# marmotlab/DCMRTA

Hardware: AMD Instinct MI355X
Metric: env_steps_per_sec (higher is better)
Workload: dtype f64

## Files before the change

### dcmrta_amd/_lib.py

```python
import ctypes as C
import os

_HERE = os.path.dirname(os.path.abspath(__file__))
LIB_PATH = os.environ.get("DCMRTA_HIP_LIB") or os.path.join(_HERE, "libdcmrta_hip.so")
HEADER_PATH = os.path.join(os.path.dirname(_HERE), "include", "dcmrta_env.h")

ABI_VERSION = 5
FOLLOWER_COLS = 4
MAX_MEMBERS = 5
MAX_MEMBERS_WIDE = 16
PARAM_NO_GROUPING, PARAM_AUTO_RESET, PARAM_STRICT_MASK, PARAM_WIDE_MEMBERS = 1, 2, 4, 8
PARAM_RENEW_SIZES = 16
POLICY_RANDOM, POLICY_FIRST, POLICY_NEAREST = 0, 1, 2
MAX_AGENTS = 128
MAX_TASKS = 1023

FLAG_DONE, FLAG_FINISHED, FLAG_TRUNCATED, FLAG_BAD_ACTION, FLAG_OVERFLOW, FLAG_BAD_LEADER, FLAG_TYPE_ERROR = 1, 2, 4, 8, 16, 32, 64
FLAG_BAD_INSTANCE = 256
FLAG_WAIT_ORDER = 128


class DcmParams(C.Structure):
    _fields_ = [("n_envs", C.c_int32), ("n_agents", C.c_int32), ("n_tasks", C.c_int32), ("device", C.c_int32),
                ("max_waiting_time", C.c_double), ("max_time", C.c_double), ("flags", C.c_uint32),
                ("auto_reset_episodes", C.c_uint32)]


class DcmError(RuntimeError):
    pass


_vp, _i32, _i64 = C.c_void_p, C.c_int32, C.c_int64
SIGNATURES = {
    "dcm_last_error": (C.c_char_p, []),
    "dcm_abi_version": (C.c_int, []),
    "dcm_build_id": (C.c_char_p, []),
    "dcm_create": (C.c_int, [C.POINTER(DcmParams), C.POINTER(_vp)]),
    "dcm_destroy": (C.c_int, [_vp]),
    "dcm_load_instances": (C.c_int, [_vp] * 6),
    "dcm_load_instances_ragged": (C.c_int, [_vp] * 8),
    "dcm_generate_instances": (C.c_int, [_vp, _vp, _i32, _i32, _i32, _i32, _i32, C.c_double, _vp]),
    "dcm_get_instances": (C.c_int, [_vp] * 8),
    "dcm_set_instance_renewal": (C.c_int, [_vp, C.c_uint64]),
    "dcm_instance_index": (C.c_int, [_vp] * 3),
    "dcm_generator_draws": (C.c_int, [_vp, _i64, _i32, C.c_uint32, _i32, _vp, _vp, _vp]),
    "dcm_reset": (C.c_int, [_vp] * 3),
    "dcm_observe": (C.c_int, [_vp] * 8),
    "dcm_step": (C.c_int, [_vp] * 11),
    "dcm_rollout_random": (C.c_int, [_vp, _i32, _i64, _vp, _vp, _vp, _vp, _vp, _vp]),
    "dcm_rollout_policy": (C.c_int, [_vp, _i32, _i32, _i64, _vp, _vp, _vp, _vp, _vp, _vp]),
    "dcm_rollout_explore": (C.c_int, [_vp, _i32, C.c_uint64, _i32, _i64, _vp, _vp, _vp, _vp, _vp, _vp]),
# ... 57 lines not shown
```

### dcmrta_amd/batched_env.py

```python
import ctypes as C
from dataclasses import dataclass

import numpy as np
import torch

from . import _lib
from ._lib import DcmError, DcmParams, check
from .choice import explore_q32 as _choice_explore_q32

SUMMARY_COLUMNS = ("reward", "n_finished", "success_rate", "makespan", "time_cost", "waiting_time", "travel_dist",
                   "efficiency")


@dataclass
class Observation:
    agents: torch.Tensor
    tasks: torch.Tensor
    mask: torch.Tensor
    leader: torch.Tensor
    active: torch.Tensor


def _ptr(t):
    return None if t is None else C.c_void_p(t.data_ptr())
# ... 74 lines not shown
            nt = np.ascontiguousarray(n_tasks, dtype=np.int32)
            na = np.ascontiguousarray(n_agents, dtype=np.int32)
            if nt.shape != (B,) or na.shape != (B,):
                raise DcmError(f"n_agents / n_tasks must be int[{B}]")
            req_np[np.arange(T)[None, :] >= nt[:, None]] = 1
        if req_np.min() < 1 or req_np.max() > self.member_cap:
            raise DcmError(f"req must be int[{B},{T}] with values in 1..{self.member_cap} (member_cap of this env)")
        d = self._dev(depot, torch.float64)
        xy = self._dev(task_xy, torch.float64)
        rq = self._dev(req, torch.int32)
        du = self._dev(dur, torch.float64)
        if d.shape != (B, 2) or xy.shape != (B, T, 2) or du.shape != (B, T):
            raise DcmError("instance arrays have the wrong shape")
        if (n_tasks is None) != (self.n_tasks is None):
            self.graph_epoch += 1
        with torch.cuda.device(self.device):
            if n_tasks is None:
                check(self._lib.dcm_load_instances(self._h, _ptr(d), _ptr(xy), _ptr(rq), _ptr(du), self._stream()))
                self.n_agents = self.n_tasks = None
            else:
                check(self._lib.dcm_load_instances_ragged(self._h, _ptr(d), _ptr(xy), _ptr(rq), _ptr(du),
                                                          na.ctypes.data_as(C.c_void_p), nt.ctypes.data_as(C.c_void_p),
                                                          self._stream()))
                self.n_agents, self.n_tasks = na.copy(), nt.copy()
        self._instances = (d, xy, rq, du)
        return self

    @staticmethod
    def _range(r, dim):
        return (dim, dim) if r is None else (int(r[0]), int(r[1])) if isinstance(r, (tuple, list)) else (int(r), int(r))

    def generate_instances(self, seeds, agents_range=None, tasks_range=None, max_coalition_size=5, max_duration=5.0):
        B = self.B
        if isinstance(seeds, (int, np.integer)):
            seeds = np.uint64(int(seeds)) + np.arange(B, dtype=np.uint64)
        if isinstance(seeds, torch.Tensor):
            if seeds.dtype not in (torch.int64, torch.uint64):
                raise DcmError("seeds must be a uint64 / int64 tensor")
            s = seeds.to(self.device).contiguous()
        else:
            s = torch.from_numpy(np.ascontiguousarray(seeds, dtype=np.uint64).view(np.int64)).to(self.device)
        if s.numel() != B:
            raise DcmError("seeds must have one entry per env")
        (a_lo, a_hi), (t_lo, t_hi) = self._range(agents_range, self.A), self._range(tasks_range, self.T)
        ragged = not (a_lo == self.A and t_lo == self.T)
        with torch.cuda.device(self.device):
            check(self._lib.dcm_generate_instances(self._h, _ptr(s), a_lo, a_hi, t_lo, t_hi, int(max_coalition_size),
                                                   float(max_duration), self._stream()))
            if ragged != (self.n_tasks is not None):
                self.graph_epoch += 1
            if ragged:
                sizes = torch.empty((2, B), dtype=torch.int32, device=self.device)
                check(self._lib.dcm_get_instances(self._h, None, None, None, None, _ptr(sizes[0]), _ptr(sizes[1]), self._stream()))
                sizes = sizes.cpu().numpy()
                self.n_agents, self.n_tasks = sizes[0].copy(), sizes[1].copy()
            else:
                self.n_agents = self.n_tasks = None
        self._instances = (s,)
        return self

    def set_instance_renewal(self, stride):
        check(self._lib.dcm_set_instance_renewal(self._h, int(stride) % (1 << 64)))
        self.graph_epoch += 1
        return self

    def instance_index(self):
        out = torch.empty((self.B,), dtype=torch.int32, device=self.device)
        with torch.cuda.device(self.device):
            check(self._lib.dcm_instance_index(self._h, _ptr(out), self._stream()))
        return out.to(torch.int64) & 0xFFFFFFFF

    def instances(self):
        B, T, dev = self.B, self.T, self.device
# ... 346 lines not shown

    def clone_state(self):
        n = C.c_size_t()
        check(self._lib.dcm_state_bytes(self._h, C.byref(n)))
        buf = torch.empty((n.value,), dtype=torch.uint8, device=self.device)
        with torch.cuda.device(self.device):
            check(self._lib.dcm_clone_state(self._h, _ptr(buf), self._stream()))
        return buf

    def restore_state(self, buf):
        n = C.c_size_t()
        check(self._lib.dcm_state_bytes(self._h, C.byref(n)))
        if buf.numel() * buf.element_size() != n.value:
            raise DcmError(f"restore_state: the snapshot holds {buf.numel() * buf.element_size()} bytes, this env's state is {n.value} "
                           "(taken from another env, or before the batch changed between uniform and ragged)")
        with torch.cuda.device(self.device):
            check(self._lib.dcm_restore_state(self._h, _ptr(buf), self._stream()))

    def fork_from(self, src, index, seeds=None, check=False):
        if not isinstance(src, BatchedTaskEnv):
            raise DcmError("fork_from: src must be a BatchedTaskEnv")
        if (src.A, src.T, src.member_cap) != (self.A, self.T, self.member_cap):
            raise DcmError(f"fork_from: src is a {src.A}A/{src.T}T env with member_cap {src.member_cap}, this one {self.A}A/{self.T}T "
                           f"with {self.member_cap}: the record layouts must be identical")
        n = index.numel() if isinstance(index, torch.Tensor) else np.asarray(index).size
        if n != self.B:
            raise DcmError(f"fork_from: index must be int32[{self.B}], one entry per env of this handle")
        if seeds is not None:
            if isinstance(seeds, torch.Tensor):
                if seeds.dtype not in (torch.int64, torch.uint64):
                    raise DcmError("fork_from: seeds must be a uint64 / int64 tensor")
                ns = seeds.numel()
            else:
                seeds = np.ascontiguousarray(seeds, dtype=np.uint64)
                ns = seeds.size
            if ns != self.B:
                raise DcmError(f"fork_from: seeds must be uint64[{self.B}], one entry per env of this handle")
        if src.device != self.device:
            raise DcmError("fork_from: the two handles are on different devices")
        if src._h is None or self._h is None:
            raise DcmError("fork_from: a handle is closed")
        idx = self._dev(index, torch.int32).reshape(-1)
        s = None
        if seeds is not None:
            s = seeds.to(self.device).contiguous() if isinstance(seeds, torch.Tensor) else torch.from_numpy(seeds.view(np.int64)).to(self.device)
        ok = torch.empty((self.B,), dtype=torch.uint8, device=self.device) if check else None
        with torch.cuda.device(self.device):
            _lib.check(self._lib.dcm_fork_envs(self._h, src._h, _ptr(idx), _ptr(s), _ptr(ok), self._stream()))
        self._fork_args = (idx, s)
        if check:
            bad = torch.nonzero(ok == 0).flatten().cpu().numpy()
            if len(bad):
                raise DcmError(f"fork_from: {len(bad)} env(s) were refused and left untouched (first: env {int(bad[0])}, index "
                               f"{int(idx[int(bad[0])])}): the index is outside [-1, {src.B}) or, in place, its source is not its own source")
        return self

    def record_bytes(self):
        n = C.c_size_t()
        check(self._lib.dcm_record_bytes(self._h, C.byref(n)))
        return n.value


group_plan = BatchedTaskEnv.group_plan
# ... 27 lines not shown
```

### dcmrta_amd/csrc/common.hpp

```cpp
#pragma once
#include <hip/hip_runtime.h>

#include <cmath>
#include <cstdint>
#include <cstdio>
#include <cstring>
#include <new>
#include <vector>

#include "../../include/dcmrta_env.h"
#include "plan.hpp"
#include "removal_table.hpp"

namespace dcm {

constexpr int WAVE = 64;
constexpr int M = DCM_MAX_MEMBERS;
constexpr int AW_MAX = (DCM_MAX_AGENTS + 63) / 64;

struct Hdr {
    double now;
    uint64_t seed;
    uint64_t d;
    double depot_x, depot_y;
// ... 294 lines not shown
__device__ double psum(const double* a, int n) {
    if constexpr (DEPTH == 0) {
        return psum_block(a, n);
    } else {
        if (n <= 128) return psum_block(a, n);
        int n2 = n / 2;
        n2 -= n2 % 8;
        return psum<DEPTH - 1>(a, n2) + psum<DEPTH - 1>(a + n2, n - n2);
    }
}

__device__ __forceinline__ double dist2(double ax, double ay, double bx, double by) {
    const double dx = ax - bx, dy = ay - by;
    return sqrt(__builtin_fma(dy, dy, dx * dx));
}
#ifndef DCM_IEEE_DIV
__device__ __forceinline__ double over_velocity(double d) {
    const double q = d * 5.0;
    const double r = __builtin_fma(-q, 0.2, d);
    return __builtin_fma(r, 5.0, q);
}
#else
__device__ __forceinline__ double over_velocity(double d) { return d / 0.2; }
#endif

__device__ __forceinline__ void copy16(unsigned char* dst, const unsigned char* src, uint32_t bytes, int lane) {
    const uint4* s = (const uint4*)src;
    uint4* d = (uint4*)dst;
    for (uint32_t i = lane; i < bytes / 16; i += WAVE) d[i] = s[i];
}
// ... 67 lines not shown
#define LAUNCH_OK() HIP_TRY(hipGetLastError())
#define GRID(env) dim3((env)->p.n_envs), dim3(dcm::WAVE)

}

struct dcm_env {
    dcm_params p;
    int A = 0, T = 0;
    dcm::Lay L;
    dcm::KP kp;
    unsigned char* state = nullptr;
    unsigned char* gscratch = nullptr;
    double* summary = nullptr;
    uint16_t* ablog = nullptr;
    bool loaded = false, reset_done = false;
    uint64_t* inst_seeds = nullptr;
    dcm::GenArgs gen{};
    bool generated = false;
    uint64_t renew_stride = 0;
    int32_t* sizes = nullptr;
    std::vector<int32_t> sizes_host;
    int32_t* routes = nullptr;
    int32_t* route_len = nullptr;
    int32_t route_cap = 0, member_cap = 0;
    double* rmarr = nullptr;
    int32_t replay_placement = 0;
    int32_t vis[4] = {20, 20, 10, 100};
    dcm::RouteLog log{nullptr, nullptr, nullptr, 0};
    dcm::RouteLog rollout_log{nullptr, nullptr, nullptr, 0};
    dcm::BestLog best_log{nullptr, nullptr, nullptr, nullptr, nullptr};
// ... 23 lines not shown
```

### dcmrta_amd/csrc/dcmrta_env.hip

```cpp
#include <array>
#include <cstdlib>
#include <mutex>
#include <tuple>
#include <type_traits>

#include "common.hpp"
#include "np_stream.hpp"

using namespace dcm;

#if defined(DCM_TU_G) || defined(DCM_TU_P) || defined(DCM_TU_L) || defined(DCM_TU_E) || defined(DCM_TU_B) || defined(DCM_TU_A)
#define DCM_DEVICE_ONLY_TU 1
#elif !defined(DCM_SPLIT_G)
#define DCM_ONE_UNIT 1
#endif
#if defined(DCM_TU_G) || defined(DCM_ONE_UNIT)
#define DCM_HAVE_FAST_G 1
#endif
#if defined(DCM_TU_P) || defined(DCM_ONE_UNIT)
#define DCM_HAVE_POLICY 1
#endif
#if defined(DCM_TU_L) || defined(DCM_ONE_UNIT)
#define DCM_HAVE_LOG 1
#endif
// ... 1246 lines not shown
        ty[t] = task_xy[((size_t)e * T + t) * 2 + 1];
        td[t] = dur[(size_t)e * T + t];
        const int32_t r = req[(size_t)e * T + t];
        bad = bad || r < 1 || r > PC;
        ti[t] = (uint32_t)(r < 1 ? 1 : r > PC ? PC : r);
    }
    bad = __any(bad);
    if (lane == 0) {
        Hdr* h = (Hdr*)rec;
        h->depot_x = depot[2 * (size_t)e]; h->depot_y = depot[2 * (size_t)e + 1];
        h->flags = DCM_FLAG_DONE | (bad ? DCM_FLAG_BAD_INSTANCE : 0u); h->episodes = 0; h->d = 0; h->seed = 0;
        h->groups = 0; h->reserved = 0; h->max_arrival = 0.0;
    }
}

template <int CA, int CT, bool RS>
constexpr uint32_t env_kernel_lds_bytes(Lay L) { return Sim<CA, CT, RS>::lds_image_bytes(L); }

template <int CA, int CT, bool RS, int MC = M>
__global__ __launch_bounds__(WAVE) void k_reset(int A, int T, int PA, int PT, KP P, unsigned char* state, const uint64_t* seeds,
                                               double* summary, uint16_t* ablog, uint32_t mode, const int32_t* sizes,
                                               unsigned char* gscr) {
    const int e = env_of_workgroup(), lane = threadIdx.x;
    int eA, eT;
    env_dims<CA, CT, RS>(sizes, e, A, T, eA, eT);
    Sim<CA, CT, RS, false, MC> S{eA, eT, PA, PT, smem, nullptr};
    const Lay L = S.L();
    S.scr = gscr + (size_t)e * L.scratch_bytes();
    unsigned char* rec = state + (size_t)e * L.rec_bytes();
    typename Sim<CA, CT, RS, false, MC>::XY xy;
// ... 254 lines not shown
    FOR_EACH_INSTANCE(SIM_CASE)
#undef SIM_CASE
    }
    return -1;
}
template <class F>
void for_each_sim(F&& f) {
#define SIM_EACH(KIND, ...) f(SimTag<__VA_ARGS__>{});
    FOR_EACH_INSTANCE(SIM_EACH)
#undef SIM_EACH
}
template <class F>
auto with_bool(bool b, F&& f) { return b ? f(std::true_type{}) : f(std::false_type{}); }
#define DIMS(env) (env)->A, (env)->T, (env)->L.A, (env)->L.T

plan::Shape shape_of(const dcm_env* env) { return {env->A, env->T, env->sizes != nullptr, env->L.C > M, env->kp.mwt > 0.0}; }
plan::SimKind sim_of(const dcm_env* env) { return plan::sim_kind(shape_of(env)); }

struct DeviceGuard {
    int prev = -1;
    explicit DeviceGuard(int dev) { if (hipGetDevice(&prev) != hipSuccess) prev = -1; if (prev != dev) (void)hipSetDevice(dev); else prev = -1; }
    ~DeviceGuard() { if (prev >= 0) (void)hipSetDevice(prev); }
};

template <class K, class... Args, class... Tail>
void launch(K kernel, unsigned grid, unsigned lds_bytes, hipStream_t stream, const std::tuple<Args...>& args, const Tail&... tail) {
    std::apply([&](const Args&... a) { hipLaunchKernelGGL(kernel, dim3(grid), dim3(WAVE), lds_bytes, stream, a..., tail...); }, args);
}
template <class... K>
void allow_lds(int bytes, K... kernels) { ((void)hipFuncSetAttribute((const void*)kernels, hipFuncAttributeMaxDynamicSharedMemorySize, bytes), ...); }

// ... 155 lines not shown

Renew renew_args(const dcm_env* env) { return Renew{env->inst_seeds, env->renew_stride, env->gen}; }
bool renew_sizes_opted_in(const dcm_env* env) { return (env->p.flags & DCM_PARAM_RENEW_SIZES) != 0; }
plan::RenewForm launch_form(const dcm_env* env) {
    return plan::renew_form(shape_of(env), env->renew_stride != 0, renew_sizes_opted_in(env));
}
plan::RenewForm renewing_launch(dcm_env* env, void* stream) {
    const plan::RenewForm form = launch_form(env);
    if (form == plan::RenewForm::Plain) return form;
    env->init_valid = false;
    if (stream_capturing(stream)) env->captured = true;
    return form;
}
void renewal_off(dcm_env* env, bool generated) { env->generated = generated; env->renew_stride = 0; }

int launch_load(dcm_env* env, const double* depot, const double* task_xy, const int32_t* req, const double* dur, void* stream) {
    hipLaunchKernelGGL(k_load_instances, GRID(env), 0, (hipStream_t)stream, DIMS(env), env->L.C, env->state, depot, task_xy,
                       req, dur, (const int32_t*)env->sizes);
    LAUNCH_OK();
    env->loaded = true;
    env->reset_done = false;
    renewal_off(env, false);
    return DCM_OK;
}

int launch_env_status(dcm_env* env, uint32_t* flags_out, int64_t* decisions_out, double* now_out, int32_t* episodes_out, void* stream) {
    const int B = env->p.n_envs;
    hipLaunchKernelGGL(k_env_status, dim3((B + WAVE - 1) / WAVE), dim3(WAVE), 0, (hipStream_t)stream, env->L.A, env->L.T, env->L.C,
                       env->state, B, flags_out, decisions_out, now_out, episodes_out);
    LAUNCH_OK();
    return DCM_OK;
}

struct Section { void* ptr; size_t bytes; };
std::array<Section, 4> state_sections(const dcm_env* env) {
    const size_t B = (size_t)env->p.n_envs;
    const bool with_sizes = env->sizes && renew_sizes_opted_in(env);
    return {{{env->state, B * env->L.rec_bytes()}, {env->summary, B * 8 * sizeof(double)},
// ... 86 lines not shown
        return fail(DCM_ERR_STATE, "%s: the best log is set and there is no best-keeping lookahead form: clear it with "
                                   "dcm_set_best_log(env, NULL, NULL, NULL, NULL, NULL)", fn);
    return rollout_form(env, fn, FORM_LOOKAHEAD, base_policy, 0, episodes, max_decisions, max_decisions_in, agents_out, tasks_out, mask_out,
                        steps_out, stream, width, inner_out);
}
}

extern "C" {

const char* dcm_last_error(void) { return dcm::g_err; }
int dcm_abi_version(void) { return DCM_ABI_VERSION; }
#ifndef DCM_BUILD_ID
#define DCM_BUILD_ID "unknown"
#endif
const char* dcm_build_id(void) { return DCM_BUILD_ID; }
#ifdef DCM_COUNT_PATHS
int dcm_debug_path_counts(unsigned long long* out32) {
    HIP_TRY(hipDeviceSynchronize());
    HIP_TRY(hipMemcpyFromSymbol(out32, HIP_SYMBOL(g_path_counts), 32 * sizeof(unsigned long long)));
    static const unsigned long long zero[32] = {};
    HIP_TRY(hipMemcpyToSymbol(HIP_SYMBOL(g_path_counts), zero, sizeof(zero)));
    return 0;
}
#endif

int dcm_create(const dcm_params* params, dcm_env** out) {
    if (!params || !out) return fail(DCM_ERR_INVALID, "dcm_create: null argument");
    *out = nullptr;
    if (params->n_envs < 1 || params->n_agents < 1 || params->n_agents > DCM_MAX_AGENTS || params->n_tasks < 1 ||
        params->n_tasks > DCM_MAX_TASKS)
// ... 60 lines not shown
    using mc = rollout_fast_mc_family;
    allow_lds(lds, mc::plain<50, 200, true>(), mc::plain<50, 200, false>(), mc::renewing<50, 200, true>(), mc::renewing<50, 200, false>());
    dcm::allow_lds_policy(lds);
    dcm::allow_lds_log(lds);
    dcm::allow_lds_explore(lds);
    dcm::allow_lds_best(lds);
    dcm::allow_lds_lookahead(lds);
    allow_lds(lds, k_get_tasks<M>, k_get_agents<M>, k_get_tasks<MW>, k_get_agents<MW>);
    return DCM_OK;
}

int dcm_destroy(dcm_env* env) {
    if (!env) return DCM_OK;
    DeviceGuard guard(env->p.device);
    void* const owned[] = {env->state, env->summary, env->ablog, env->gscratch, env->routes, env->route_len,
                           env->rmarr, env->sizes, env->side, env->pendq, env->init, env->inst_seeds, env->la_snap};
    for (void* p : owned)
        if (p) (void)hipFree(p);
    delete env;
    return DCM_OK;
}

int dcm_load_instances(dcm_env* env, const double* depot, const double* task_xy, const int32_t* req, const double* dur,
                       void* stream) {
    CHECK_ENV(env);
    if (!depot || !task_xy || !req || !dur) return fail(DCM_ERR_INVALID, "dcm_load_instances: null array");
    DCM_TRY(dcm::drop_pending(env, stream));
    if (env->sizes) { HIP_TRY(hipFree(env->sizes)); env->sizes = nullptr; }
    return launch_load(env, depot, task_xy, req, dur, stream);
}

// ... 29 lines not shown
    DCM_TRY(dcm::drop_pending(env, stream));
    renewal_off(env, false);
    const bool uniform = agents_lo == env->A && tasks_lo == env->T;
    if (uniform && env->sizes) { HIP_TRY(hipFree(env->sizes)); env->sizes = nullptr; }
    if (!uniform && !env->sizes) HIP_TRY(hipMalloc((void**)&env->sizes, (size_t)2 * env->p.n_envs * sizeof(int32_t)));
    const size_t seed_bytes = (size_t)env->p.n_envs * sizeof(uint64_t);
    if (!env->inst_seeds) HIP_TRY(hipMalloc((void**)&env->inst_seeds, seed_bytes));
    HIP_TRY(hipMemcpyAsync(env->inst_seeds, inst_seeds, seed_bytes, hipMemcpyDeviceToDevice, (hipStream_t)stream));
    const GenArgs g{agents_lo, agents_hi, tasks_lo, tasks_hi, max_coalition_size, max_duration};
    hipLaunchKernelGGL(k_generate_instances, GRID(env), 0, (hipStream_t)stream, env->L.A, env->L.T, env->L.C, env->state, inst_seeds, g,
                       env->sizes);
    LAUNCH_OK();
    env->loaded = true;
    env->reset_done = false;
    env->gen = g;
    renewal_off(env, true);
    return DCM_OK;
}

int dcm_get_instances(dcm_env* env, double* depot, double* task_xy, int32_t* req, double* dur, int32_t* n_agents, int32_t* n_tasks,
                      void* stream) {
    CHECK_ENV(env);
    if (!env->loaded) return fail(DCM_ERR_STATE, "dcm_get_instances: no instances loaded");
    hipLaunchKernelGGL(k_get_instances, GRID(env), 0, (hipStream_t)stream, DIMS(env), env->L.C, (const unsigned char*)env->state,
                       (const int32_t*)env->sizes, depot, task_xy, req, dur, n_agents, n_tasks);
    LAUNCH_OK();
    return DCM_OK;
}

int dcm_set_instance_renewal(dcm_env* env, uint64_t stride) {
// ... 248 lines not shown
        if (e->renew_stride != 0)
            return fail(DCM_ERR_STATE, "dcm_fork_envs: %s has a renewal stride set: clear it with dcm_set_instance_renewal(env, 0) first", which);
    }
    DCM_TRY(dcm::flush_pending(src, stream));
    if (dst != src) DCM_TRY(dcm::flush_pending(dst, stream));
    const Lay& L = dst->L;
    const uint32_t log_bytes = (uint32_t)dst->A * AB_CAP * sizeof(uint16_t), cnt_bytes = (uint32_t)abcnt_pitch(dst->A, dst->T);
    unsigned char* const cnt_dst = (unsigned char*)dst->ablog + (size_t)dst->p.n_envs * log_bytes;
    const unsigned char* const cnt_src = (const unsigned char*)src->ablog + (size_t)src->p.n_envs * log_bytes;
    hipLaunchKernelGGL(k_fork_envs, GRID(dst), 0, (hipStream_t)stream, src->p.n_envs, dst == src, L.rec_bytes() / 16, log_bytes / 16, cnt_bytes / 16,
                       dst->state, (const unsigned char*)src->state, dst->summary, (const double*)src->summary, (unsigned char*)dst->ablog,
                       (const unsigned char*)src->ablog, cnt_dst, cnt_src, src_index, seeds_in, ok_out);
    LAUNCH_OK();
    dst->init_valid = false;
    renewal_off(dst, false);
    return DCM_OK;
}

int dcm_rollout_random(dcm_env* env, int32_t episodes, int64_t max_decisions, const int64_t* max_decisions_in,
                       float* agents_out, float* tasks_out, uint8_t* mask_out, int64_t* steps_out, void* stream) {
    CHECK_ENV(env);
    if (!env->reset_done) return fail(DCM_ERR_STATE, "dcm_rollout_random: call dcm_reset first");
    if (episodes < 1) return fail(DCM_ERR_INVALID, "dcm_rollout_random: episodes must be >= 1");
    if (env->rollout_log.len || env->best_log.episode)
        return rollout_form(env, "dcm_rollout_random", form_of(env, FORM_LOG), DCM_POLICY_RANDOM, 0, episodes, max_decisions, max_decisions_in, agents_out,
                            tasks_out, mask_out, steps_out, stream);
    DCM_TRY(dcm::flush_pending(env, stream));
    const plan::RenewForm form = renewing_launch(env, stream);
    const dcm::RolloutArgs ra = rollout_args(env, form, episodes, max_decisions, max_decisions_in, agents_out, tasks_out, mask_out, steps_out);
    const auto args = ra.kernel_args();
// ... 164 lines not shown
}

int dcm_restore_state(dcm_env* env, const void* src, void* stream) {
    CHECK_ENV(env);
    if (!src) return fail(DCM_ERR_INVALID, "dcm_restore_state: null src");
    DCM_TRY(dcm::drop_pending(env, stream));
    const unsigned char* in = (const unsigned char*)src;
    for (const Section& s : state_sections(env)) {
        if (s.bytes == 0) continue;
        HIP_TRY(hipMemcpyAsync(s.ptr, in, s.bytes, hipMemcpyDeviceToDevice, (hipStream_t)stream));
        in += s.bytes;
    }
    env->loaded = true;
    env->reset_done = true;
    env->init_valid = false;
    return DCM_OK;
}

int dcm_distance(const double* ax, const double* ay, const double* bx, const double* by, double* dist_out, double* time_out,
                 int64_t n, void* stream) {
    if (!ax || !ay || !bx || !by || n < 0) return fail(DCM_ERR_INVALID, "dcm_distance: bad argument");
    if (n == 0) return DCM_OK;
    hipLaunchKernelGGL(k_distance, dim3((unsigned)((n + 255) / 256)), dim3(256), 0, (hipStream_t)stream, ax, ay, bx, by,
                       dist_out, time_out, n);
    LAUNCH_OK();
    return DCM_OK;
}

#ifdef DCM_PROFILE_PHASES
int dcm_prof_read_fast(unsigned long long* out16, int reset) {
    HIP_TRY(hipDeviceSynchronize());
// ... 27 lines not shown
```

### dcmrta_amd/csrc/k_rollout_fast.inc

```
#define KBASE rollout_fast
#define KPOLICY_FORMS 1
#include "k_form.inc"
template <int CA, int CT, bool RS, bool OBS, bool PRIO = false>
__global__ __launch_bounds__(WAVE, 4) void KNAME(int A, int T, int PA, int PT, KP P, unsigned char* state, int episodes,
                                                      float* agents_out, float* tasks_out, uint8_t* mask_out,
                                                      int64_t* steps_out, double* summary, uint16_t* ablog,
                                                      KSIZES, int64_t budget_all, const int64_t* budget_in,
                                                      unsigned char* gscr, double* retlog, int retcap KRENEW_PARAM KPOLICY_PARAM) {
    const int e = env_of_workgroup(), lane = threadIdx.x;
    int eA, eT;
    env_dims<CA, CT, RS>(sizes, e, A, T, eA, eT);
    using F = Fast<CA, CT, RS, OBS>;
    using SimT = typename F::SimT;
    SimT S{eA, eT, PA, PT, smem, nullptr};
    const Lay L = S.L();
    S.scr = SimT::SCR_IN_LDS ? smem + L.lds_rec() : gscr + (size_t)e * L.scratch_bytes();
    const int BA = S.BA(A), BT = S.BT(T);
    unsigned char* rec = state + (size_t)e * L.rec_bytes();
    typename SimT::XY xy;
    S.template load_record<true, false>(rec, lane, xy);
    S.set_ablog(ablog, e, BA, BT, lane);
    S.set_retlog(retlog, retcap, e, lane);
    WSYNC();
    HdrRegs h = load_hdr(smem);
// ... 101 lines not shown
#endif
                h.flags &= ~SimT::FLAG_DEFERRED;
            }
#endif
            need_adv = 0;
            h.now = uni(h.now); h.flags = uni(h.flags); h.cur_group = uni(h.cur_group); h.n_groups = uni(h.n_groups);
            h.empty_passes = uni(h.empty_passes);
        }
        if (!(h.flags & DCM_FLAG_DONE) && left != 0) {
            WSYNC();
            f.reload(r);
            FPHK(f, 13);
            for (;;) {
                FPHK(f, 12);
                CNT(0);
                const uint64_t k1 = rl(kv, ki), k2 = rl(kv2, ki);
#ifdef KEXPLORES
                const bool explores = x_all || rl(xv, ki) < x_q;
                const int rlen = f.decide_logged(r, h, P, lane, k1, agrow, tkrow, mkp, &k2, explores ? DCM_POLICY_RANDOM : policy, fl);
#elif defined(DCM_LOG)
                const int rlen = f.decide_logged(r, h, P, lane, k1, agrow, tkrow, mkp, &k2, policy, fl);
#elif defined(DCM_POLICY)
                const int rlen = f.decide_policy(r, h, P, lane, k1, agrow, tkrow, mkp, &k2, policy);
#else
                const int rlen = f.decide(r, h, P, lane, k1, agrow, tkrow, mkp, &k2, use_prio ? &nv_last : nullptr);
#endif
#ifdef KEXPLORES
                if (h.flags & DCM_FLAG_DONE) break;
#else
                int more = 0;
                uint32_t done = h.flags & DCM_FLAG_DONE;
// ... 70 lines not shown
```

### dcmrta_amd/csrc/plan.hpp

```cpp
#pragma once
#include <cstdint>

#include "../../include/dcmrta_env.h"

namespace dcm::plan {

constexpr int LANES = 64;

struct Shape { int A, T; bool ragged, wide, quiet; };

struct LayDims { int A, T, C; };
inline LayDims layout_dims(int A, int T, bool wide) {
    if (wide) return {A, T, DCM_MAX_MEMBERS_WIDE};
    if (A <= 20 && T <= 50) return {20, 50, DCM_MAX_MEMBERS};
    if (A <= LANES && T <= LANES) return {LANES, LANES, DCM_MAX_MEMBERS};
    return {A, T, DCM_MAX_MEMBERS};
}

enum class SimKind { S20x50, S20x50_RS, S64x64_RS, S50x200, S100x500, S128x256_RS, Runtime, RuntimeWide };
inline SimKind sim_kind(const Shape& s) {
    const bool uniform = !s.ragged;
    if (s.wide) return SimKind::RuntimeWide;
    if (s.A <= 20 && s.T <= 50) return (uniform && s.A == 20 && s.T == 50) ? SimKind::S20x50 : SimKind::S20x50_RS;
    if (s.A <= LANES && s.T <= LANES) return SimKind::S64x64_RS;
    if (uniform && s.A == 50 && s.T == 200) return SimKind::S50x200;
    if (uniform && s.A == 100 && s.T == 500) return SimKind::S100x500;
    if (s.A <= 2 * LANES && s.T <= 4 * LANES) return SimKind::S128x256_RS;
    return SimKind::Runtime;
}

inline bool one_chunk_ok(const Shape& s) { return s.quiet && !s.wide && s.A <= LANES && s.T <= LANES - 1; }

inline bool renewal_ok(const Shape& s, bool generated) { return generated && !s.ragged; }
inline bool renewal_sizes_ok(const Shape& s, bool generated, bool opted_in) { return generated && opted_in && s.ragged; }
enum class RenewForm { Plain, Instance, Sizes };
inline RenewForm renew_form(const Shape& s, bool stride_set, bool opted_in) {
    if (!stride_set) return RenewForm::Plain;
    return (s.ragged && opted_in) ? RenewForm::Sizes : RenewForm::Instance;
}
inline bool defer_terminal(bool captured, RenewForm form) { return !captured && form != RenewForm::Sizes; }
inline bool step_restart_image(bool image_valid, bool deferred_terminal, bool renewal) { return image_valid && deferred_terminal && !renewal; }

enum class Rollout { Fast, FastMc, FastG, General };
inline Rollout rollout_kind(const Shape& s, bool obs_all_or_none) {
    if (!s.quiet || s.wide || !obs_all_or_none) return Rollout::General;
    if (one_chunk_ok(s)) return Rollout::Fast;
// ... 29 lines not shown
```

### dcmrta_amd/csrc/rollout_fast.hpp

```cpp
#pragma once
#include <type_traits>

struct FastLog {
    int16_t* task;
    double* arrival;
    int32_t cap;
    int32_t len;
};

template <int CA, int CT, bool RS, bool OBS, bool TRK = false>
struct Fast {
    using SimT = Sim<CA, CT, RS, false>;
    using AMask = typename SimT::AMask;
    static_assert(CA >= 1 && CA <= 64 && CT >= 1 && CT <= 64, "one lane per agent / task; lane 63 is the depot's (the host dispatches T <= 63 only)");
    static constexpr int DL = 63;
    static constexpr Lay L{CA, CT};

    SimT S;
    uint4* rtab;
    mutable uint32_t dirty = 0;
    mutable uint64_t achg = ~0ull;
    mutable uint64_t dt_join = 0, dt_times = 0;
    mutable uint64_t unsettled = ~0ull;
    FPH_MEMBERS;
// ... 128 lines not shown
                    *(double*)((unsigned char*)row0 + off[j]) = av[j];
                }
                gone = (uint64_t)g;
                r.ids = (uint64_t)__builtin_amdgcn_perm(idh, idl, e.x);
                r.lm &= ~gone;
                nn = (int)(e.w >> 16);
                r.nab += (uint32_t)(n - nn);
            }
            if constexpr (TRK) dirty |= SimT::DIRTY_ALL & ~SimT::DIRTY_TIMES;
            uint64_t todo = dmask;
            do {
                CNT(7);
                const int t = __ffsll((unsigned long long)todo) - 1;
                todo &= todo - 1ull;
                const uint64_t g = rl(gone, t);
                if (lane_of(g)) {
                    const uint32_t nth_ = r.ai >> 16;
                    r.ai += 1u << 16;
                    if (nth_ < (uint32_t)AB_CAP) ((__attribute__((address_space(1))) uint16_t*)r.ab)[nth_] = (uint16_t)t;
                    else {
                        const uint32_t ci = (uint32_t)(la * S.T() + t);
                        __hip_atomic_fetch_add((__attribute__((address_space(1))) uint32_t*)S.abcnt() + (ci >> 1), 1u << (16 * (ci & 1)),
                                               __ATOMIC_RELAXED, __HIP_MEMORY_SCOPE_AGENT);
                    }
                    if (r.cur == t) r.ai &= ~A_MEMBER;
                }
            } while (todo);
            FPM(21);
        }
        const uint32_t info_i = ((info | (ok ? T_FEAS : 0u)) & (T_FEAS | T_FIN | 0xFFu)) | ((uint32_t)(status & 0xFF) << 8) | ((uint32_t)nn << 16);
        const uint32_t info_f = info | ((now >= tfin) ? T_FIN : 0u);
        info = feas0 ? info_f : info_i;
        r.ti = info;
        if (inT) S.tinfo()[lt] = info;
        uint64_t over_already = 0ull;
        if (bec) {
            r.ts = nts; r.tf = ntf;
            if (inT) { S.ts()[lt] = nts; S.tf()[lt] = ntf; }
            if constexpr (TRK) { dirty |= SimT::DIRTY_TIMES; dt_times |= bec; }
// ... 51 lines not shown
        gm = __ballot((int)((r.ai >> 8) & 0xFFu) == h.cur_group) & am;
        const int glen = __popcll(gm);
        if (glen == 0) return -1;
        return nth(gm, below((uint32_t)(k1 >> 32), glen));
    }
    __device__ __forceinline__ int pick_leader_flagged(const R& r, HdrRegs& h, uint64_t k1, uint64_t& gm) const {
        const uint64_t g = __ballot((int)((r.ai >> 8) & 0xFFu) == h.cur_group) & am;
        int glen = __popcll(g);
        asm("" : "+s"(glen));
        const uint32_t bad = (uint32_t)((glen - 1) >> 31);
        gm = g | (uint64_t)(bad & 1u);
        h.flags |= bad & (uint32_t)(DCM_FLAG_BAD_LEADER | DCM_FLAG_DONE);
        return nth(gm, below((uint32_t)(k1 >> 32), glen + (int)(bad & 1u)));
    }
    __device__ __forceinline__ int decide(R& r, HdrRegs& h, const KP& P, int lane, uint64_t k1, float* agrow, float* tkrow, uint8_t* mkp,
                                          const uint64_t* k2p = nullptr, int* nvp = nullptr) const {
        uint64_t gm;
        const int leader = pick_leader_flagged(r, h, k1, gm);
        FPH(0);
        const uint64_t bm = observe(r, h.now, leader, agrow, tkrow, mkp);
        FPH(1);
        int nv = __popcll(bm);
        asm("" : "+s"(nv));
        if (nvp) *nvp = nv;
        const int drawn = nth(bm, below((uint32_t)k1, nv)) + 1;
        const int action = nv ? drawn : 0;
        FPH(2);
        return apply(r, h, P, lane, k1, gm, leader, action, k2p);
    }
    __device__ __forceinline__ int decide_policy(R& r, HdrRegs& h, const KP& P, int lane, uint64_t k1, float* agrow, float* tkrow, uint8_t* mkp,
                                                 const uint64_t* k2p, int policy) const {
        uint64_t gm;
        const int leader = pick_leader_flagged(r, h, k1, gm);
        FPH(0);
        const uint64_t bm = observe(r, h.now, leader, agrow, tkrow, mkp);
        FPH(1);
        uint64_t pick = bm;
        if (policy == DCM_POLICY_NEAREST) {
            const double lx = rl(r.ax, leader), ly = rl(r.ay, leader);
            const double dd = dist2(lx, ly, r.tx, r.ty);
            const bool open = lane_of(bm);
            const double m = wave_nanmin_n<CT>(open ? dd : __builtin_nan(""));
            pick = bm & __ballot(dd == m);
        }
        const int action = __ffsll((unsigned long long)pick);
        FPH(2);
        return apply(r, h, P, lane, k1, gm, leader, action, k2p);
    }
    __device__ __forceinline__ int decide_logged(R& r, HdrRegs& h, const KP& P, int lane, uint64_t k1, float* agrow, float* tkrow, uint8_t* mkp,
                                                 const uint64_t* k2p, int policy, FastLog& lg) const {
        uint64_t gm;
        const int leader = pick_leader_flagged(r, h, k1, gm);
        FPH(0);
        const uint64_t bm = observe(r, h.now, leader, agrow, tkrow, mkp);
        FPH(1);
        int nv = __popcll(bm);
        asm("" : "+s"(nv));
        const int drawn = nth(bm, below((uint32_t)k1, nv)) + 1;
        uint64_t pick = bm;
        if (policy == DCM_POLICY_NEAREST) {
            const double lx = rl(r.ax, leader), ly = rl(r.ay, leader);
            const double dd = dist2(lx, ly, r.tx, r.ty);
            const bool open = lane_of(bm);
            const double m = wave_nanmin_n<CT>(open ? dd : __builtin_nan(""));
            pick = bm & __ballot(dd == m);
        }
        const int greedy = __ffsll((unsigned long long)pick);
        int pol = policy;
        asm("" : "+s"(pol));
        const int action = pol == DCM_POLICY_RANDOM ? (nv ? drawn : 0) : greedy;
        FPH(2);
        return apply<true>(r, h, P, lane, k1, gm, leader, action, k2p, &lg);
    }
    template <bool LOG = false>
    __device__ __forceinline__ int apply(R& r, const HdrRegs& h, const KP& P, int lane, uint64_t k1, uint64_t gm, int leader, int action,
                                         const uint64_t* k2p = nullptr, FastLog* lg = nullptr) const {
        const double now = h.now;
        uint64_t rest = gm & ~(1ull << leader);
        int rlen = __popcll(gm) - 1;
        uint64_t mm = 1ull << leader, mlist = (uint64_t)(uint32_t)leader;
        int nm = 1;
        int mypos = 0;
        action = uni(action);
        int task = action - 1;
        asm("" : "+s"(task));
        int act_ = action;
        asm("" : "+s"(act_));
        auto go = [&]() __attribute__((always_inline)) { int c = act_; asm("" : "+s"(c)); return c != 0; };
        static_assert(DL == 63, "task & DL");
        const int tl = task & DL;
        if (!go()) {
            CNT(2);
            mm |= rest; nm += rlen; rlen = 0;
        } else if (rlen != 0) {
            const int vacancy = (int)(int8_t)(((uint32_t)__builtin_amdgcn_readlane((int)r.ti, tl) >> 8) & 0xFF);
            const int nf = (vacancy > 1) ? ((vacancy - 1 < rlen) ? vacancy - 1 : rlen) : 0;
            uint64_t kk = k1;
            auto draw = [&](uint32_t rr) {
                CNT(1);
                FPM(22);
                const int f = nth(rest, below(rr, rlen));
                rest &= ~(1ull << f); rlen--;
                mm |= 1ull << f;
                mlist |= (uint64_t)(uint32_t)f << (8 * nm);
                mypos = lane == f ? nm : mypos;
                nm++;
                FPM(23);
            };
            for (int j = 0; j < nf; j += 2) {
                kk = (j == 0 && k2p) ? *k2p : mix64(kk + GAMMA);
                draw((uint32_t)(kk >> 32));
                if (j + 1 < nf) draw((uint32_t)kk);
            }
        }
        FPH(3);
        const double tx_ = rl(r.tx, tl), ty_ = rl(r.ty, tl);
        double d = dist2(r.ax, r.ay, tx_, ty_);
        double arrv = now + over_velocity(d);
        asm volatile("" : "+v"(d), "+v"(arrv));
        FPH(4);
        const bool mem = lane_of(mm);
        uint64_t ids = 0ull; uint32_t kinfo = 0; int n = 0;
        int slot = 0;
        if (go()) {
            kinfo = (uint32_t)__builtin_amdgcn_readlane((int)r.ti, tl);
            ids = rl(r.ids, tl);
            n = (kinfo >> 16) & 0xFF;
            slot = n + mypos;
            if constexpr (TRK) {
                dirty |= SimT::DIRTY_IDS | ((rl(r.lm, tl) & mm) ? SimT::DIRTY_ROWS : ((((1u << nm) - 1u) << (n + 1)) & SimT::DIRTY_ROWS));
                dt_join |= 1ull << tl;
            }
            if (rl(r.lm, tl) & mm) {
                CNT(3);
                for (int j = 0; j < nm; j++) {
                    const int m = (int)((mlist >> (8 * j)) & 0xFF);
                    const uint64_t x = ids ^ (0x0101010101010101ull * (uint64_t)(uint32_t)m);
                    uint64_t z = (x - 0x0101010101010101ull) & ~x & 0x8080808080808080ull;
                    z &= (n >= 8) ? ~0ull : ((1ull << (8 * n)) - 1ull);
                    int pos;
// ... 107 lines not shown
```

### include/dcmrta_env.h

```cpp
#ifndef DCMRTA_ENV_H
#define DCMRTA_ENV_H

#include <stddef.h>
#include <stdint.h>

#ifdef __cplusplus
extern "C" {
#endif

#define DCM_ABI_VERSION 5

typedef struct dcm_env dcm_env;

typedef enum {
    DCM_OK = 0,
    DCM_ERR_INVALID = -1,
    DCM_ERR_HIP = -2,
    DCM_ERR_NO_DEVICE = -3,
    DCM_ERR_STATE = -4
} dcm_status;

#define DCM_MAX_AGENTS 128
#define DCM_MAX_TASKS 1023
#define DCM_MAX_MEMBERS 5
// ... 24 lines not shown
    double max_waiting_time;
    double max_time;
    uint32_t flags;
    uint32_t auto_reset_episodes;
} dcm_params;

const char *dcm_last_error(void);
int dcm_abi_version(void);
const char *dcm_build_id(void);

int dcm_create(const dcm_params *params, dcm_env **out);
int dcm_destroy(dcm_env *env);

int dcm_load_instances(dcm_env *env, const double *depot, const double *task_xy, const int32_t *req,
                       const double *dur, void *stream);

int dcm_load_instances_ragged(dcm_env *env, const double *depot, const double *task_xy, const int32_t *req,
                              const double *dur, const int32_t *n_agents, const int32_t *n_tasks, void *stream);

int dcm_generate_instances(dcm_env *env, const uint64_t *inst_seeds, int32_t agents_lo, int32_t agents_hi, int32_t tasks_lo,
                           int32_t tasks_hi, int32_t max_coalition_size, double max_duration, void *stream);

int dcm_get_instances(dcm_env *env, double *depot, double *task_xy, int32_t *req, double *dur, int32_t *n_agents,
                      int32_t *n_tasks, void *stream);

int dcm_set_instance_renewal(dcm_env *env, uint64_t stride);
int dcm_instance_index(dcm_env *env, uint32_t *index_out, void *stream);

int dcm_generator_draws(const uint64_t *seeds, int64_t n, int32_t n_doubles, uint32_t bound, int32_t n_ints,
                        double *doubles_out, uint32_t *ints_out, void *stream);
// ... 91 lines not shown
```

Baseline: 1.703 billion.

## Use fast rsq-based sqrt in rollout fast path with range validation and key readlane deferral

Replaces the IEEE sqrt in the fast rollout distance computation with a cheaper hardware reciprocal-square-root plus Newton refinement, valid only when squared distances are not tiny. The change adds a host-side validation kernel that runs at instance load or restore and falls back to the general kernels when any point pair is too close, which costs a sync there. It also defers the second key readlane until it is actually used, hoists a duplicated readlane of task info, and turns the abandonment log write into a ballot-based branch. A kernel-name query lets the Python side bump graph_epoch when kernel selection changes.

```diff
diff --git a/dcmrta_amd/_lib.py b/dcmrta_amd/_lib.py
--- a/dcmrta_amd/_lib.py
+++ b/dcmrta_amd/_lib.py
@@ -12,6 +12,7 @@
 PARAM_NO_GROUPING, PARAM_AUTO_RESET, PARAM_STRICT_MASK, PARAM_WIDE_MEMBERS = 1, 2, 4, 8
 PARAM_RENEW_SIZES = 16
 POLICY_RANDOM, POLICY_FIRST, POLICY_NEAREST = 0, 1, 2
+KERNEL_ROLLOUT, KERNEL_STEP = 0, 1
 MAX_AGENTS = 128
 MAX_TASKS = 1023
 
@@ -35,6 +36,7 @@
     "dcm_last_error": (C.c_char_p, []),
     "dcm_abi_version": (C.c_int, []),
     "dcm_build_id": (C.c_char_p, []),
+    "dcm_kernel_name": (C.c_char_p, [_vp, _i32]),
     "dcm_create": (C.c_int, [C.POINTER(DcmParams), C.POINTER(_vp)]),
     "dcm_destroy": (C.c_int, [_vp]),
     "dcm_load_instances": (C.c_int, [_vp] * 6),
diff --git a/dcmrta_amd/batched_env.py b/dcmrta_amd/batched_env.py
--- a/dcmrta_amd/batched_env.py
+++ b/dcmrta_amd/batched_env.py
@@ -112,6 +112,7 @@
             raise DcmError("instance arrays have the wrong shape")
         if (n_tasks is None) != (self.n_tasks is None):
             self.graph_epoch += 1
+        kernels = self._kernel_names()
         with torch.cuda.device(self.device):
             if n_tasks is None:
                 check(self._lib.dcm_load_instances(self._h, _ptr(d), _ptr(xy), _ptr(rq), _ptr(du), self._stream()))
@@ -122,7 +123,24 @@
                                                           self._stream()))
                 self.n_agents, self.n_tasks = na.copy(), nt.copy()
         self._instances = (d, xy, rq, du)
-        return self
+        self._kernels_since(kernels)
+        return self
+
+    def kernel_name(self, entry="rollout"):
+        which = {"rollout": _lib.KERNEL_ROLLOUT, "step": _lib.KERNEL_STEP}.get(entry)
+        if which is None:
+            raise DcmError('kernel_name: entry is "rollout" or "step"')
+        name = self._lib.dcm_kernel_name(self._h, which)
+        if name is None:
+            check(-1)
+        return name.decode()
+
+    def _kernel_names(self):
+        return self.kernel_name("rollout"), self.kernel_name("step")
+
+    def _kernels_since(self, before):
+        if self._kernel_names() != before:
+            self.graph_epoch += 1
 
     @staticmethod
     def _range(r, dim):
@@ -142,6 +160,7 @@
             raise DcmError("seeds must have one entry per env")
         (a_lo, a_hi), (t_lo, t_hi) = self._range(agents_range, self.A), self._range(tasks_range, self.T)
         ragged = not (a_lo == self.A and t_lo == self.T)
+        kernels = self._kernel_names()
         with torch.cuda.device(self.device):
             check(self._lib.dcm_generate_instances(self._h, _ptr(s), a_lo, a_hi, t_lo, t_hi, int(max_coalition_size),
                                                    float(max_duration), self._stream()))
@@ -155,6 +174,7 @@
             else:
                 self.n_agents = self.n_tasks = None
         self._instances = (s,)
+        self._kernels_since(kernels)
         return self
 
     def set_instance_renewal(self, stride):
@@ -531,8 +551,10 @@
         if buf.numel() * buf.element_size() != n.value:
             raise DcmError(f"restore_state: the snapshot holds {buf.numel() * buf.element_size()} bytes, this env's state is {n.value} "
                            "(taken from another env, or before the batch changed between uniform and ragged)")
+        kernels = self._kernel_names()
         with torch.cuda.device(self.device):
             check(self._lib.dcm_restore_state(self._h, _ptr(buf), self._stream()))
+        self._kernels_since(kernels)
 
     def fork_from(self, src, index, seeds=None, check=False):
         if not isinstance(src, BatchedTaskEnv):
@@ -562,8 +584,10 @@
         if seeds is not None:
             s = seeds.to(self.device).contiguous() if isinstance(seeds, torch.Tensor) else torch.from_numpy(seeds.view(np.int64)).to(self.device)
         ok = torch.empty((self.B,), dtype=torch.uint8, device=self.device) if check else None
+        kernels = self._kernel_names()
         with torch.cuda.device(self.device):
             _lib.check(self._lib.dcm_fork_envs(self._h, src._h, _ptr(idx), _ptr(s), _ptr(ok), self._stream()))
+        self._kernels_since(kernels)
         self._fork_args = (idx, s)
         if check:
             bad = torch.nonzero(ok == 0).flatten().cpu().numpy()
diff --git a/dcmrta_amd/csrc/common.hpp b/dcmrta_amd/csrc/common.hpp
--- a/dcmrta_amd/csrc/common.hpp
+++ b/dcmrta_amd/csrc/common.hpp
@@ -332,6 +332,21 @@
     const double dx = ax - bx, dy = ay - by;
     return sqrt(__builtin_fma(dy, dy, dx * dx));
 }
+constexpr double DIST2_INRANGE_MIN = 0x1p-767;
+__device__ __forceinline__ double dist2_inrange(double ax, double ay, double bx, double by) {
+    const double dx = ax - bx, dy = ay - by;
+    const double x = __builtin_fma(dy, dy, dx * dx);
+    const double y = __builtin_amdgcn_rsq(x);
+    double g = x * y, h = y * 0.5;
+    const double e = __builtin_fma(-h, g, 0.5);
+    g = __builtin_fma(g, e, g);
+    h = __builtin_fma(h, e, h);
+    g = __builtin_fma(__builtin_fma(-g, g, x), h, g);
+    g = __builtin_fma(__builtin_fma(-g, g, x), h, g);
+    int zero_or_inf = 0x260;
+    asm("" : "+s"(zero_or_inf));
+    return __builtin_amdgcn_class(x, zero_or_inf) ? x : g;
+}
 #ifndef DCM_IEEE_DIV
 __device__ __forceinline__ double over_velocity(double d) {
     const double q = d * 5.0;
@@ -429,6 +444,8 @@
     double* summary = nullptr;
     uint16_t* ablog = nullptr;
     bool loaded = false, reset_done = false;
+    bool inrange = true;
+    uint32_t* inrange_bad = nullptr;
     uint64_t* inst_seeds = nullptr;
     dcm::GenArgs gen{};
     bool generated = false;
diff --git a/dcmrta_amd/csrc/dcmrta_env.hip b/dcmrta_amd/csrc/dcmrta_env.hip
--- a/dcmrta_amd/csrc/dcmrta_env.hip
+++ b/dcmrta_amd/csrc/dcmrta_env.hip
@@ -1284,6 +1284,29 @@
     }
 }
 
+#ifndef DCM_DEVICE_ONLY_TU
+__global__ __launch_bounds__(WAVE) void k_points_inrange(int A, int T, int PA, int PT, int PC, const unsigned char* state, const int32_t* sizes,
+                                                        uint32_t* bad) {
+    const int e = blockIdx.x, lane = threadIdx.x;
+    int eA, eT;
+    env_dims<0, 0, false>(sizes, e, A, T, eA, eT);
+    const Lay L{PA, PT, PC};
+    const unsigned char* rec = state + (size_t)e * L.rec_bytes();
+    const double *tx = (const double*)(rec + L.tx()), *ty = (const double*)(rec + L.ty());
+    const Hdr* h = (const Hdr*)rec;
+    bool out = false;
+    for (int j = lane; j < eT; j += WAVE) {
+        const double bx = tx[j], by = ty[j];
+        for (int i = -1; i < j; i++) {
+            const double dx = (i < 0 ? h->depot_x : tx[i]) - bx, dy = (i < 0 ? h->depot_y : ty[i]) - by;
+            const double q = __builtin_fma(dy, dy, dx * dx);
+            out = out || (q > 0.0 && q < DIST2_INRANGE_MIN);
+        }
+    }
+    if (__any(out) && lane == 0) atomicOr(bad, 1u);
+}
+#endif
+
 template <int CA, int CT, bool RS>
 constexpr uint32_t env_kernel_lds_bytes(Lay L) { return Sim<CA, CT, RS>::lds_image_bytes(L); }
 
@@ -1568,7 +1591,7 @@
 auto with_bool(bool b, F&& f) { return b ? f(std::true_type{}) : f(std::false_type{}); }
 #define DIMS(env) (env)->A, (env)->T, (env)->L.A, (env)->L.T
 
-plan::Shape shape_of(const dcm_env* env) { return {env->A, env->T, env->sizes != nullptr, env->L.C > M, env->kp.mwt > 0.0}; }
+plan::Shape shape_of(const dcm_env* env) { return {env->A, env->T, env->sizes != nullptr, env->L.C > M, env->kp.mwt > 0.0, env->inrange}; }
 plan::SimKind sim_of(const dcm_env* env) { return plan::sim_kind(shape_of(env)); }
 
 struct DeviceGuard {
@@ -1754,6 +1777,23 @@
 }
 void renewal_off(dcm_env* env, bool generated) { env->generated = generated; env->renew_stride = 0; }
 
+int check_points_inrange(dcm_env* env, void* stream) {
+    env->inrange = true;
+    if (!plan::one_chunk_ok(shape_of(env))) return DCM_OK;
+    env->inrange = false;
+    if (stream_capturing(stream)) return DCM_OK;
+    if (!env->inrange_bad) HIP_TRY(hipMalloc((void**)&env->inrange_bad, sizeof(uint32_t)));
+    HIP_TRY(hipMemsetAsync(env->inrange_bad, 0, sizeof(uint32_t), (hipStream_t)stream));
+    hipLaunchKernelGGL(k_points_inrange, GRID(env), 0, (hipStream_t)stream, DIMS(env), env->L.C, (const unsigned char*)env->state,
+                       (const int32_t*)env->sizes, env->inrange_bad);
+    LAUNCH_OK();
+    uint32_t bad = 1;
+    HIP_TRY(hipMemcpyAsync(&bad, env->inrange_bad, sizeof(uint32_t), hipMemcpyDeviceToHost, (hipStream_t)stream));
+    HIP_TRY(hipStreamSynchronize((hipStream_t)stream));
+    env->inrange = bad == 0;
+    return DCM_OK;
+}
+
 int launch_load(dcm_env* env, const double* depot, const double* task_xy, const int32_t* req, const double* dur, void* stream) {
     hipLaunchKernelGGL(k_load_instances, GRID(env), 0, (hipStream_t)stream, DIMS(env), env->L.C, env->state, depot, task_xy,
                        req, dur, (const int32_t*)env->sizes);
@@ -1761,7 +1801,7 @@
     env->loaded = true;
     env->reset_done = false;
     renewal_off(env, false);
-    return DCM_OK;
+    return check_points_inrange(env, stream);
 }
 
 int launch_env_status(dcm_env* env, uint32_t* flags_out, int64_t* decisions_out, double* now_out, int32_t* episodes_out, void* stream) {
@@ -1878,6 +1918,18 @@
 #define DCM_BUILD_ID "unknown"
 #endif
 const char* dcm_build_id(void) { return DCM_BUILD_ID; }
+const char* dcm_kernel_name(dcm_env* env, int32_t entry) {
+    if (!env) { (void)dcm::fail(DCM_ERR_INVALID, "null env handle"); return nullptr; }
+    const plan::Shape shape = shape_of(env);
+    if (entry == DCM_KERNEL_STEP) return plan::one_chunk_ok(shape) ? "k_step_fast" : "k_step";
+    if (entry != DCM_KERNEL_ROLLOUT) { (void)dcm::fail(DCM_ERR_INVALID, "dcm_kernel_name: unknown entry"); return nullptr; }
+    switch (plan::rollout_kind(shape, true)) {
+    case plan::Rollout::Fast: return "k_rollout_fast";
+    case plan::Rollout::FastMc: return "k_rollout_fast_mc";
+    case plan::Rollout::FastG: return "k_rollout_fast_g";
+    default: return "k_rollout_random";
+    }
+}
 #ifdef DCM_COUNT_PATHS
 int dcm_debug_path_counts(unsigned long long* out32) {
     HIP_TRY(hipDeviceSynchronize());
@@ -1968,7 +2020,7 @@
     if (!env) return DCM_OK;
     DeviceGuard guard(env->p.device);
     void* const owned[] = {env->state, env->summary, env->ablog, env->gscratch, env->routes, env->route_len,
-                           env->rmarr, env->sizes, env->side, env->pendq, env->init, env->inst_seeds, env->la_snap};
+                           env->rmarr, env->sizes, env->side, env->pendq, env->init, env->inst_seeds, env->la_snap, env->inrange_bad};
     for (void* p : owned)
         if (p) (void)hipFree(p);
     delete env;
@@ -2028,6 +2080,7 @@
     env->loaded = true;
     env->reset_done = false;
     env->gen = g;
+    env->inrange = true;
     renewal_off(env, true);
     return DCM_OK;
 }
@@ -2306,6 +2359,7 @@
     LAUNCH_OK();
     dst->init_valid = false;
     renewal_off(dst, false);
+    dst->inrange = dst->inrange && src->inrange;
     return DCM_OK;
 }
 
@@ -2500,7 +2554,7 @@
     env->loaded = true;
     env->reset_done = true;
     env->init_valid = false;
-    return DCM_OK;
+    return check_points_inrange(env, stream);
 }
 
 int dcm_distance(const double* ax, const double* ay, const double* bx, const double* by, double* dist_out, double* time_out,
diff --git a/dcmrta_amd/csrc/k_rollout_fast.inc b/dcmrta_amd/csrc/k_rollout_fast.inc
--- a/dcmrta_amd/csrc/k_rollout_fast.inc
+++ b/dcmrta_amd/csrc/k_rollout_fast.inc
@@ -139,7 +139,8 @@
             for (;;) {
                 FPHK(f, 12);
                 CNT(0);
-                const uint64_t k1 = rl(kv, ki), k2 = rl(kv2, ki);
+                const uint64_t k1 = rl(kv, ki);
+                const Key2 k2{kv2, ki};
 #ifdef KEXPLORES
                 const bool explores = x_all || rl(xv, ki) < x_q;
                 const int rlen = f.decide_logged(r, h, P, lane, k1, agrow, tkrow, mkp, &k2, explores ? DCM_POLICY_RANDOM : policy, fl);
diff --git a/dcmrta_amd/csrc/plan.hpp b/dcmrta_amd/csrc/plan.hpp
--- a/dcmrta_amd/csrc/plan.hpp
+++ b/dcmrta_amd/csrc/plan.hpp
@@ -7,7 +7,7 @@
 
 constexpr int LANES = 64;
 
-struct Shape { int A, T; bool ragged, wide, quiet; };
+struct Shape { int A, T; bool ragged, wide, quiet; bool inrange = true; };
 
 struct LayDims { int A, T, C; };
 inline LayDims layout_dims(int A, int T, bool wide) {
@@ -29,7 +29,7 @@
     return SimKind::Runtime;
 }
 
-inline bool one_chunk_ok(const Shape& s) { return s.quiet && !s.wide && s.A <= LANES && s.T <= LANES - 1; }
+inline bool one_chunk_ok(const Shape& s) { return s.quiet && s.inrange && !s.wide && s.A <= LANES && s.T <= LANES - 1; }
 
 inline bool renewal_ok(const Shape& s, bool generated) { return generated && !s.ragged; }
 inline bool renewal_sizes_ok(const Shape& s, bool generated, bool opted_in) { return generated && opted_in && s.ragged; }
diff --git a/dcmrta_amd/csrc/rollout_fast.hpp b/dcmrta_amd/csrc/rollout_fast.hpp
--- a/dcmrta_amd/csrc/rollout_fast.hpp
+++ b/dcmrta_amd/csrc/rollout_fast.hpp
@@ -6,6 +6,11 @@
     double* arrival;
     int32_t cap;
     int32_t len;
+};
+
+struct Key2 {
+    uint64_t kv2;
+    int ki;
 };
 
 template <int CA, int CT, bool RS, bool OBS, bool TRK = false>
@@ -166,15 +171,19 @@
                 const int t = __ffsll((unsigned long long)todo) - 1;
                 todo &= todo - 1ull;
                 const uint64_t g = rl(gone, t);
-                if (lane_of(g)) {
-                    const uint32_t nth_ = r.ai >> 16;
-                    r.ai += 1u << 16;
-                    if (nth_ < (uint32_t)AB_CAP) ((__attribute__((address_space(1))) uint16_t*)r.ab)[nth_] = (uint16_t)t;
-                    else {
+                const uint64_t room = g & __ballot(r.ai < ((uint32_t)AB_CAP << 16));
+                const uint32_t nth_ = r.ai >> 16;
+                if (lane_of(room)) ((__attribute__((address_space(1))) uint16_t*)r.ab)[nth_] = (uint16_t)t;
+                const uint64_t over = g & ~room;
+                if (over) {
+                    if (lane_of(over)) {
                         const uint32_t ci = (uint32_t)(la * S.T() + t);
                         __hip_atomic_fetch_add((__attribute__((address_space(1))) uint32_t*)S.abcnt() + (ci >> 1), 1u << (16 * (ci & 1)),
                                                __ATOMIC_RELAXED, __HIP_MEMORY_SCOPE_AGENT);
                     }
+                }
+                if (lane_of(g)) {
+                    r.ai += 1u << 16;
                     if (r.cur == t) r.ai &= ~A_MEMBER;
                 }
             } while (todo);
@@ -256,7 +265,7 @@
         return nth(gm, below((uint32_t)(k1 >> 32), glen + (int)(bad & 1u)));
     }
     __device__ __forceinline__ int decide(R& r, HdrRegs& h, const KP& P, int lane, uint64_t k1, float* agrow, float* tkrow, uint8_t* mkp,
-                                          const uint64_t* k2p = nullptr, int* nvp = nullptr) const {
+                                          const Key2* k2p = nullptr, int* nvp = nullptr) const {
         uint64_t gm;
         const int leader = pick_leader_flagged(r, h, k1, gm);
         FPH(0);
@@ -271,7 +280,7 @@
         return apply(r, h, P, lane, k1, gm, leader, action, k2p);
     }
     __device__ __forceinline__ int decide_policy(R& r, HdrRegs& h, const KP& P, int lane, uint64_t k1, float* agrow, float* tkrow, uint8_t* mkp,
-                                                 const uint64_t* k2p, int policy) const {
+                                                 const Key2* k2p, int policy) const {
         uint64_t gm;
         const int leader = pick_leader_flagged(r, h, k1, gm);
         FPH(0);
@@ -280,7 +289,7 @@
         uint64_t pick = bm;
         if (policy == DCM_POLICY_NEAREST) {
             const double lx = rl(r.ax, leader), ly = rl(r.ay, leader);
-            const double dd = dist2(lx, ly, r.tx, r.ty);
+            const double dd = dist2_inrange(lx, ly, r.tx, r.ty);
             const bool open = lane_of(bm);
             const double m = wave_nanmin_n<CT>(open ? dd : __builtin_nan(""));
             pick = bm & __ballot(dd == m);
@@ -290,7 +299,7 @@
         return apply(r, h, P, lane, k1, gm, leader, action, k2p);
     }
     __device__ __forceinline__ int decide_logged(R& r, HdrRegs& h, const KP& P, int lane, uint64_t k1, float* agrow, float* tkrow, uint8_t* mkp,
-                                                 const uint64_t* k2p, int policy, FastLog& lg) const {
+                                                 const Key2* k2p, int policy, FastLog& lg) const {
         uint64_t gm;
         const int leader = pick_leader_flagged(r, h, k1, gm);
         FPH(0);
@@ -302,7 +311,7 @@
         uint64_t pick = bm;
         if (policy == DCM_POLICY_NEAREST) {
             const double lx = rl(r.ax, leader), ly = rl(r.ay, leader);
-            const double dd = dist2(lx, ly, r.tx, r.ty);
+            const double dd = dist2_inrange(lx, ly, r.tx, r.ty);
             const bool open = lane_of(bm);
             const double m = wave_nanmin_n<CT>(open ? dd : __builtin_nan(""));
             pick = bm & __ballot(dd == m);
@@ -316,7 +325,7 @@
     }
     template <bool LOG = false>
     __device__ __forceinline__ int apply(R& r, const HdrRegs& h, const KP& P, int lane, uint64_t k1, uint64_t gm, int leader, int action,
-                                         const uint64_t* k2p = nullptr, FastLog* lg = nullptr) const {
+                                         const Key2* k2p = nullptr, FastLog* lg = nullptr) const {
         const double now = h.now;
         uint64_t rest = gm & ~(1ull << leader);
         int rlen = __popcll(gm) - 1;
@@ -331,11 +340,12 @@
         auto go = [&]() __attribute__((always_inline)) { int c = act_; asm("" : "+s"(c)); return c != 0; };
         static_assert(DL == 63, "task & DL");
         const int tl = task & DL;
+        const uint32_t tiw = (uint32_t)__builtin_amdgcn_readlane((int)r.ti, tl);
         if (!go()) {
             CNT(2);
             mm |= rest; nm += rlen; rlen = 0;
         } else if (rlen != 0) {
-            const int vacancy = (int)(int8_t)(((uint32_t)__builtin_amdgcn_readlane((int)r.ti, tl) >> 8) & 0xFF);
+            const int vacancy = (int)(int8_t)((tiw >> 8) & 0xFF);
             const int nf = (vacancy > 1) ? ((vacancy - 1 < rlen) ? vacancy - 1 : rlen) : 0;
             uint64_t kk = k1;
             auto draw = [&](uint32_t rr) {
@@ -350,14 +360,14 @@
                 FPM(23);
             };
             for (int j = 0; j < nf; j += 2) {
-                kk = (j == 0 && k2p) ? *k2p : mix64(kk + GAMMA);
+                kk = (j == 0 && k2p) ? rl(k2p->kv2, k2p->ki) : mix64(kk + GAMMA);
                 draw((uint32_t)(kk >> 32));
                 if (j + 1 < nf) draw((uint32_t)kk);
             }
         }
         FPH(3);
         const double tx_ = rl(r.tx, tl), ty_ = rl(r.ty, tl);
-        double d = dist2(r.ax, r.ay, tx_, ty_);
+        double d = dist2_inrange(r.ax, r.ay, tx_, ty_);
         double arrv = now + over_velocity(d);
         asm volatile("" : "+v"(d), "+v"(arrv));
         FPH(4);
@@ -365,7 +375,7 @@
         uint64_t ids = 0ull; uint32_t kinfo = 0; int n = 0;
         int slot = 0;
         if (go()) {
-            kinfo = (uint32_t)__builtin_amdgcn_readlane((int)r.ti, tl);
+            kinfo = tiw;
             ids = rl(r.ids, tl);
             n = (kinfo >> 16) & 0xFF;
             slot = n + mypos;
diff --git a/include/dcmrta_env.h b/include/dcmrta_env.h
--- a/include/dcmrta_env.h
+++ b/include/dcmrta_env.h
@@ -62,6 +62,10 @@
 
 int dcm_load_instances(dcm_env *env, const double *depot, const double *task_xy, const int32_t *req,
                        const double *dur, void *stream);
+
+#define DCM_KERNEL_ROLLOUT 0
+#define DCM_KERNEL_STEP 1
+const char *dcm_kernel_name(dcm_env *env, int32_t entry);
 
 int dcm_load_instances_ragged(dcm_env *env, const double *depot, const double *task_xy, const int32_t *req,
                               const double *dur, const int32_t *n_agents, const int32_t *n_tasks, void *stream);
```

New measurement: 1.749 billion, median of 6. 1.03x the previous value.
